# szemenyeim/DynEnv

Hardware: AMD Instinct MI355X
Metric: agent-steps/s (higher is better)
Workload: dtype f64

## Files before the change

### dynenv_amd/csrc/dev_common.h

```cpp
#pragma once
#include <hip/hip_runtime.h>
#include <stdint.h>

#include "dynenv.h"
#include "dynenv_math.h"

#define DE_WAVE 64
#define DE_DEV __device__ __forceinline__
#define DE_OOL static __device__ __noinline__
#define DE_HD __host__ __device__ __forceinline__

struct V2 {
  double x, y;
};
DE_HD V2 v2(double x, double y) { V2 r; r.x = x; r.y = y; return r; }
DE_HD V2 vadd(V2 a, V2 b) { return v2(a.x + b.x, a.y + b.y); }
DE_HD V2 vsub(V2 a, V2 b) { return v2(a.x - b.x, a.y - b.y); }
DE_HD V2 vneg(V2 a) { return v2(-a.x, -a.y); }
DE_HD V2 vmul(V2 a, double s) { return v2(a.x * s, a.y * s); }
DE_HD double vdot(V2 a, V2 b) { return a.x * b.x + a.y * b.y; }
DE_HD double vcross(V2 a, V2 b) { return a.x * b.y - a.y * b.x; }
DE_HD V2 vperp(V2 a) { return v2(-a.y, a.x); }
DE_HD V2 vrotate(V2 a, V2 b) { return v2(a.x * b.x - a.y * b.y, a.x * b.y + a.y * b.x); }
DE_HD double vdot_f(V2 a, V2 b) { return dms_dot(a.x, a.y, b.x, b.y); }
DE_HD V2 vrotate_f(V2 n, V2 j) { return v2(dms_rotate_x(n.x, n.y, j.x, j.y), dms_rotate_y(n.x, n.y, j.x, j.y)); }
DE_HD double vlensq(V2 a) { return vdot(a, a); }
DE_HD V2 vlerp(V2 a, V2 b, double t) { return vadd(vmul(a, 1.0 - t), vmul(b, t)); }
DE_HD double vlen(V2 v) { return dm_sqrt(v.x * v.x + v.y * v.y); }
DE_HD V2 vrot_angle(V2 v, double a) {
  double s, c;
  dm_sincos(a, &s, &c);
  return v2(v.x * c - v.y * s, v.x * s + v.y * c);
}
DE_HD double fmax_cp(double a, double b) { return (a > b) ? a : b; }
DE_HD double fmin_cp(double a, double b) { return (a < b) ? a : b; }
DE_HD double fclamp_cp(double f, double lo, double hi) { return fmin_cp(fmax_cp(f, lo), hi); }
DE_HD double fclamp01_cp(double f) { return fmax_cp(0.0, fmin_cp(f, 1.0)); }

DE_DEV uint64_t wave_ballot(bool p) { return __ballot(p); }
DE_DEV int lane_id() { return (int)__builtin_amdgcn_mbcnt_hi(~0u, __builtin_amdgcn_mbcnt_lo(~0u, 0u)); }
DE_DEV int fresh_lane() {
  int l;
  asm volatile("v_mbcnt_lo_u32_b32 %0, -1, 0\n\tv_mbcnt_hi_u32_b32 %0, -1, %0" : "=v"(l));
  return l;
}
DE_DEV uint64_t lanemask_lt() { return (1ull << lane_id()) - 1ull; }

DE_DEV int bcast_i(int v, int src) { return __builtin_amdgcn_readlane(v, __builtin_amdgcn_readfirstlane(src)); }
DE_DEV double bcast_d(double v, int src) {
  union { double d; int i[2]; } u;
  u.d = v;
  src = __builtin_amdgcn_readfirstlane(src);
  u.i[0] = __builtin_amdgcn_readlane(u.i[0], src);
  u.i[1] = __builtin_amdgcn_readlane(u.i[1], src);
  return u.d;
}
DE_DEV int lane_read_i(int v, int src) { return __builtin_amdgcn_ds_bpermute(src << 2, v); }
DE_DEV double lane_read_d(double v, int src) {
  union { double d; int i[2]; } u;
  u.d = v;
  u.i[0] = __builtin_amdgcn_ds_bpermute(src << 2, u.i[0]);
  u.i[1] = __builtin_amdgcn_ds_bpermute(src << 2, u.i[1]);
  return u.d;
}
DE_DEV int uniform_i(int v) { return __builtin_amdgcn_readfirstlane(v); }
DE_DEV uint64_t uniform_u64(uint64_t v) {
  uint32_t lo = (uint32_t)__builtin_amdgcn_readfirstlane((int)(uint32_t)v);
  uint32_t hi = (uint32_t)__builtin_amdgcn_readfirstlane((int)(uint32_t)(v >> 32));
  return ((uint64_t)hi << 32) | lo;
}
template <typename T>
DE_DEV T* uniform_ptr(T* p) { return (T*)uniform_u64((uint64_t)p); }
DE_DEV double uniform_d(double v) { return __longlong_as_double((long long)uniform_u64((uint64_t)__double_as_longlong(v))); }

struct DevSC {
  double s, c;
};
DE_OOL DevSC dev_sincos(double x) {
  DevSC r;
  dm_sincos(x, &r.s, &r.c);
  return r;
}
DE_OOL DevSC dev_sincos_v(double x) {
  DevSC r;
  dm_sincos_f(x, &r.s, &r.c);
  return r;
}
DE_DEV DevSC dev_sincos_inl(double x) {
  DevSC r;
  dm_sincos(x, &r.s, &r.c);
  return r;
}
DE_OOL double dev_atan2(double y, double x) { return dm_atan2(y, x); }
__device__ const double g_atanTab[30] = DM_ATAN_TAB;
#define DEV_ATAN_TAB_INIT(dst, lane) do { if ((lane) < 30) (dst)[lane] = g_atanTab[lane]; } while (0)
DE_DEV int dev_lds_addr(const void* p) { return (int)(size_t)(const __attribute__((address_space(3))) void*)p; }
DE_OOL double dev_atan2_t(double y, double x, int tab) {
  typedef double __attribute__((ext_vector_type(2))) d2;
  const double aq = __builtin_fabs(y / x);
  typedef const __attribute__((address_space(3))) d2* lds_d2p;
  const lds_d2p row = (lds_d2p)(size_t)(unsigned)(tab + 48 * dm_atan_row(aq));
  const d2 n = row[0], d = row[1], hl = row[2];
  return dm_atan2_finish(y, x, aq, dm_atan_core(aq, n.x, n.y, d.x, d.y, hl.x, hl.y));
}
DE_DEV double dev_cos(double x) { return dev_sincos(x).c; }

#define DE_DBL_MIN 2.2250738585072014e-308
#define DE_COLLISION_SLOP 0.1
#define DE_CONTACT_BIAS_COEF 0.061259621561307376
#define DE_PIVOT_BIAS_COEF 0.022762779044189331
#define DE_JOINT_BIAS_COEF DE_CONTACT_BIAS_COEF
#define DE_DT 0.01
```

### dynenv_amd/csrc/driving_kernels.hip

```cpp
#include "driving_dev.h"

__constant__ DrvConst C;

#include "driving_host.h"

struct DrvMailbox {
  double p1x[DRV_NS][2], p1y[DRV_NS][2], p2x[DRV_NS][2], p2y[DRV_NS][2], nx[DRV_NS], ny[DRV_NS];
  int hash[DRV_NS][2], count[DRV_NS], flag[DRV_NS];
};
struct DrvObsStage {
  float carRow[DRV_MAXA][8];
  float goal[DRV_MAXA][2];
  float shared[DRV_MAXO * 4 + DRV_MAXP * 2 + DRV_LANE_ROWS * 5];
};
#ifdef DRV_PROFILE
#define DRV_PROF(...) __VA_ARGS__
#else
#define DRV_PROF(...)
#endif
#define DRV_CLIST 128
struct __align__(16) DrvLds {
  double px[DRV_NB], py[DRV_NB], vx[DRV_NB], vy[DRV_NB], ang[DRV_NB], w[DRV_NB], vbx[DRV_NB], vby[DRV_NB], wb[DRV_NB];
  double minv[DRV_NB], iinv[DRV_NB];
  double rc[16], rs[16], rotAng[16];
// ... 73 lines not shown
    double relAngle = cosRel * dist;
    pos = relAngle < 0.0 ? LP_InRightLane : LP_InOpposingLane;
  }
  return pos;
}

DE_DEV bool drv_is_off_road(V2 point) {
  int position = LP_OffRoad;
  int rp = road_pos<0>(point, RoadK<0>::cosDir0);
  if (rp < position) position = rp;
  rp = road_pos<1>(point, RoadK<1>::cosDir0);
  if (rp < position) position = rp;
  return position >= LP_OverRoad;
}
DE_DEV bool drv_is_out(V2 p) { return p.x <= 0.0 || p.y <= 0.0 || p.x >= DRV_W || p.y >= DRV_H; }

DE_DEV void apply_friction(double& vx, double& vy, double& w, double m, double friction, double rotFriction,
                           double spin) {
  vx = vx * 1.0 + (0.0 + 0.0) * DE_DT;
  vy = vy * 1.0 + (0.0 + 0.0) * DE_DT;
  w = w * 1.0 + 0.0;
  double factor = friction * m;
  double rotFactor = rotFriction * m;
  double x = vx, y = vy;
  double length = 1.0 / (dm_abs(x) + dm_abs(y) + 1e-5);
  double theta = w;
  double a0 = x * factor * length;
  double a1 = y * factor * length;
  a0 += a1 * spin * theta;
  a1 -= a0 * spin * theta;
  if (dm_abs(x) < factor) x = 0.0; else x -= a0;
  if (dm_abs(y) < factor) y = 0.0; else y -= a1;
  if (dm_abs(theta) < rotFactor) theta = 0.0; else theta -= (theta > 0.0 ? rotFactor : -rotFactor);
  vx = x; vy = y; w = theta;
}

DE_DEV void velocity_update(DrvLds& L, int lane, bool isCar, bool isPed) {
  if (!(isCar || isPed)) return;
  double vx = L.vx[lane], vy = L.vy[lane], w = L.w[lane];
  const int f = L.flags[lane];
  double m, fr, rfr;
  bool dflt = false;
  if (isCar) { m = L.cmass[lane]; fr = CF_FRIC(f) ? 5e-4 : 5e-5; rfr = CF_FRIC(f) ? 2e-5 : 1e-5; }
  else { m = 90.0; fr = 5e-2; rfr = 2e-4; dflt = !PF_DEAD(f); }
  if (dflt) { vx = vx * 1.0 + (0.0 + 0.0) * DE_DT; vy = vy * 1.0 + (0.0 + 0.0) * DE_DT; w = w * 1.0 + 0.0; }
  else apply_friction(vx, vy, w, m, fr, rfr, 0.0);
  L.vx[lane] = vx; L.vy[lane] = vy; L.w[lane] = w;
}
DE_OOL void velocity_update_ool(int nCarPed) {
  const int lane = lane_id(), A = uniform_i(nCarPed) & 0xFF, nPed = uniform_i(nCarPed) >> 8;
  velocity_update(g_L, lane, lane < A, lane >= DRV_SLOT_PED && lane < DRV_SLOT_PED + nPed);
}

struct CarRot { double c, s, cosRel0; };
template <bool INL = false>
DE_DEV CarRot car_refresh_rot(DrvLds& L, int lane, double ang) {
  const DevSC sc = INL ? dev_sincos_inl(ang) : dev_sincos(ang);
  CarRot r;
  r.c = sc.c; r.s = sc.s;
  r.cosRel0 = INL ? dev_sincos_inl(RoadK<0>::dirAngle - ang).c : dev_cos(RoadK<0>::dirAngle - ang);
  L.rc[lane] = r.c; L.rs[lane] = r.s; L.rotAng[lane] = ang; L.cosRel0[lane] = r.cosRel0;
  static_assert(RoadK<1>::dirAngle == 0.0, "cos(road1.dirAngle - angle) is read from rc");
  return r;
}

struct BoxW {
  V2 v[4], n[4];
};
DE_DEV void box_world(BoxW& b, V2 p, double rc, double rs, double hx, double hy) {
  const double lx[4] = {-hx, hx, hx, -hx}, ly[4] = {-hy, -hy, hy, hy};
  const double nx[4] = {-1.0, 0.0, 1.0, 0.0}, ny[4] = {0.0, -1.0, 0.0, 1.0};
#pragma unroll
  for (int i = 0; i < 4; ++i) {
    b.v[i] = v2(dms_xform_x(rc, rs, lx[i], ly[i], p.x), dms_xform_y(rc, rs, lx[i], ly[i], p.y));
    b.n[i] = v2(rc * nx[i] - rs * ny[i], rs * nx[i] + rc * ny[i]);
  }
}

struct Contacts {
  int count;
  V2 n, p1[2], p2[2];
  int hash[2];
};

struct EdgeW {
  V2 ap, bp, n;
  int ah, bh;
};

DE_DEV V2 sel4(const V2* a, int i) {
  V2 r = a[0];
  r = (i == 1) ? a[1] : r;
  r = (i == 2) ? a[2] : r;
  r = (i == 3) ? a[3] : r;
  return r;
}

struct BoxP {
  V2 p;
  double c, s, hx, hy;
};
DE_DEV V2 boxp_vertex(const BoxP& b, int i) {
  const double lx = (i == 1 || i == 2) ? b.hx : -b.hx;
  const double ly = (i >= 2) ? b.hy : -b.hy;
  return v2(dms_xform_x(b.c, b.s, lx, ly, b.p.x), dms_xform_y(b.c, b.s, lx, ly, b.p.y));
}
DE_DEV V2 boxp_normal(const BoxP& b, int i) {
  const double nx = (i == 0) ? -1.0 : ((i == 2) ? 1.0 : 0.0);
  const double ny = (i == 1) ? -1.0 : ((i == 3) ? 1.0 : 0.0);
  return v2(b.c * nx - b.s * ny, b.s * nx + b.c * ny);
}

template <int S> DE_DEV double quad_bcast(double x) {
  int lo = __double2loint(x), hi = __double2hiint(x);
  lo = __builtin_amdgcn_update_dpp(lo, lo, S * 0x55, 0xF, 0xF, false);
  hi = __builtin_amdgcn_update_dpp(hi, hi, S * 0x55, 0xF, 0xF, false);
  return __hiloint2double(hi, lo);
}
DE_DEV void quad_argmax_first(double v, double& best, int& idx) {
  best = -INFINITY; idx = 0;
  double m;
  m = quad_bcast<0>(v); if (m > best) { best = m; idx = 0; }
  m = quad_bcast<1>(v); if (m > best) { best = m; idx = 1; }
  m = quad_bcast<2>(v); if (m > best) { best = m; idx = 2; }
  m = quad_bcast<3>(v); if (m > best) { best = m; idx = 3; }
}

DE_DEV int poly_support_index(const BoxP& p, V2 n, int q) {
  double mx;
  int index;
  quad_argmax_first(vdot_f(boxp_vertex(p, q), n), mx, index);
  return index;
}

DE_DEV EdgeW support_edge_poly(const BoxP& p, int slot, V2 n, int q) {
  int i1 = poly_support_index(p, n, q);
  int i0 = (i1 + 3) & 3;
  int i2 = (i1 + 1) & 3;
  int h = slot * 4;
  V2 n1 = boxp_normal(p, i1), n2 = boxp_normal(p, i2);
  EdgeW e;
  V2 vm = boxp_vertex(p, i1);
  if (vdot(n, n1) > vdot(n, n2)) {
    e.ap = boxp_vertex(p, i0); e.ah = h + i0; e.bp = vm; e.bh = h + i1; e.n = n1;
  } else {
    e.ap = vm; e.ah = h + i1; e.bp = boxp_vertex(p, i2); e.bh = h + i2; e.n = n2;
  }
  return e;
}

DE_DEV int hash_pair(int a, int b) { return 1 + ((a << 8) | b); }

DE_DEV void contact_points(const EdgeW& e1, const EdgeW& e2, V2 n, Contacts& out) {
  double d_e1_a = vcross(e1.ap, n), d_e1_b = vcross(e1.bp, n);
  double d_e2_a = vcross(e2.ap, n), d_e2_b = vcross(e2.bp, n);
  double e1_denom = 1.0 / (d_e1_b - d_e1_a + DE_DBL_MIN);
  double e2_denom = 1.0 / (d_e2_b - d_e2_a + DE_DBL_MIN);
  out.n = n;
  out.count = 0;
  {
    V2 p1 = vadd(vmul(n, 0.0), vlerp(e1.ap, e1.bp, fclamp01_cp((d_e2_b - d_e1_a) * e1_denom)));
    V2 p2 = vadd(vmul(n, -0.0), vlerp(e2.ap, e2.bp, fclamp01_cp((d_e1_a - d_e2_a) * e2_denom)));
    double dist = vdot(vsub(p2, p1), n);
    if (dist <= 0.0) { out.p1[0] = p1; out.p2[0] = p2; out.hash[0] = hash_pair(e1.ah, e2.bh); out.count = 1; }
  }
  {
    V2 p1 = vadd(vmul(n, 0.0), vlerp(e1.ap, e1.bp, fclamp01_cp((d_e2_a - d_e1_a) * e1_denom)));
    V2 p2 = vadd(vmul(n, -0.0), vlerp(e2.ap, e2.bp, fclamp01_cp((d_e1_b - d_e2_a) * e2_denom)));
    double dist = vdot(vsub(p2, p1), n);
    if (dist <= 0.0) {
      int h = hash_pair(e1.bh, e2.ah);
      if (out.count == 0) { out.p1[0] = p1; out.p2[0] = p2; out.hash[0] = h; }
      else { out.p1[1] = p1; out.p2[1] = p2; out.hash[1] = h; }
      out.count += 1;
    }
  }
}

DE_DEV double sat_max_sep(const BoxP& a, const BoxP& b, int q, int& best) {
  const V2 n = boxp_normal(a, q);
  const double d0 = vdot_f(n, boxp_vertex(a, q));
  double minv = INFINITY;
#pragma unroll
  for (int j = 0; j < 4; ++j) {
    double d = vdot_f(n, boxp_vertex(b, j)) - d0;
    if (d < minv) minv = d;
  }
  double maxsep;
  quad_argmax_first(minv, maxsep, best);
  return maxsep;
}

DE_DEV void poly_to_poly(const BoxP& p1, int slot1, const BoxP& p2, int slot2, int q, Contacts& out) {
  out.count = 0;
  int ia, ib;
  double sa = sat_max_sep(p1, p2, q, ia);
  if (sa > 0.0) return;
  double sb = sat_max_sep(p2, p1, q, ib);
  if (sb > 0.0) return;
  V2 n;
  if (sa >= sb) n = boxp_normal(p1, ia); else n = vneg(boxp_normal(p2, ib));
  const EdgeW e1 = support_edge_poly(p1, slot1, n, q);
  const EdgeW e2 = support_edge_poly(p2, slot2, vneg(n), q);
  contact_points(e1, e2, n, out);
}

DE_DEV void circle_to_poly(V2 c, double r, const BoxP& poly, int q, Contacts& out) {
  out.count = 0;
  double maxsep;
  int best;
  const V2 vq = boxp_vertex(poly, q);
  quad_argmax_first(vdot(boxp_normal(poly, q), vsub(c, vq)), maxsep, best);
  if (maxsep > r) return;
  if (maxsep <= 0.0) {
    V2 fn = boxp_normal(poly, best);
    V2 n = vneg(fn);
    V2 pb = vsub(c, vmul(fn, maxsep));
    out.n = n; out.p1[0] = vadd(c, vmul(n, r)); out.p2[0] = pb; out.hash[0] = 0; out.count = 1;
  } else {
    const V2 a = boxp_vertex(poly, (q + 3) & 3), b = vq;
    const V2 d = vsub(b, a);
    const double t = fclamp01_cp(vdot(d, vsub(c, a)) / vlensq(d));
    const V2 pt = vadd(a, vmul(d, t));
    const double dsq = vlensq(vsub(pt, c));
    double bestd = INFINITY;
    V2 bestp = c;
    double m;
    m = quad_bcast<0>(dsq); if (m < bestd) { bestd = m; bestp = v2(quad_bcast<0>(pt.x), quad_bcast<0>(pt.y)); }
    m = quad_bcast<1>(dsq); if (m < bestd) { bestd = m; bestp = v2(quad_bcast<1>(pt.x), quad_bcast<1>(pt.y)); }
    m = quad_bcast<2>(dsq); if (m < bestd) { bestd = m; bestp = v2(quad_bcast<2>(pt.x), quad_bcast<2>(pt.y)); }
    m = quad_bcast<3>(dsq); if (m < bestd) { bestd = m; bestp = v2(quad_bcast<3>(pt.x), quad_bcast<3>(pt.y)); }
    if (bestd <= r * r) {
      double dist = dm_sqrt(bestd);
      V2 delta = vsub(bestp, c);
      V2 n = (dist != 0.0) ? vmul(delta, 1.0 / dist) : vneg(boxp_normal(poly, best));
      out.n = n; out.p1[0] = vadd(c, vmul(n, r)); out.p2[0] = bestp; out.hash[0] = 0; out.count = 1;
    }
  }
}

struct BodyV {
  V2 p, v, vb;
  double w, wb, minv, iinv;
};
DE_DEV V2 static_pos(const DrvLds& L, int idx) {
  if (idx >= DRV_SLOT_BLD) {
    int k = idx - DRV_SLOT_BLD;
    return v2((k & 2) ? 1385.0 : 365.0, (k & 1) ? 800.0 : 200.0);
  }
  return v2(L.ox[idx - DRV_SLOT_OBST], L.oy[idx - DRV_SLOT_OBST]);
}
DE_DEV void body_load(const DrvLds& L, int idx, BodyV& b) {
  const bool dyn = idx < DRV_SLOT_OBST;
  const int bi = dyn ? idx : DRV_SLOT_OBST , oi = (idx >= DRV_SLOT_OBST && idx < DRV_SLOT_BLD) ? idx - DRV_SLOT_OBST : 0;
  const double dpx = L.px[bi], dpy = L.py[bi], sox = L.ox[oi], soy = L.oy[oi];
  const int k = idx - DRV_SLOT_BLD;
// ... 373 lines not shown
    const V2 jl = vmul(n, dj);                                                              \
    const V2 jj = biasLane ? jl : jr;                                                       \
    apply_impulse(a, vneg(jj), r1[q]);                                                      \
    apply_impulse(b, jj, r2[q]);                                                            \
  }
  for (int t = 0; t < nSteps; ++t) {
    if (active && t == due && passes < 10) {
      a.v = v2(fX[ra], fY[ra]); a.w = fW[ra];
      b.v = v2(fX[rb], fY[rb]); b.w = fW[rb];
      DRV_SPLIT_PASS(0)
      if (count > 1) DRV_SPLIT_PASS(1)
      fX[wa] = a.v.x; fY[wa] = a.v.y; fW[wa] = a.w;
      fX[wb_] = b.v.x; fY[wb_] = b.v.y; fW[wb_] = b.w;
      due += period; ++passes;
    }
    __syncthreads();
  }
#undef DRV_SPLIT_PASS
  DrvSplitRet r;
  r.jt0 = jt0; r.jt1 = jt1; r.pk = pk; r.pair = pair; r.bits = bits3;
  r.jn0 = acc[0]; r.jn1 = acc[1];
  r.jb0 = lane_read_d(acc[0], (lane + 32) & 63); r.jb1 = lane_read_d(acc[1], (lane + 32) & 63);
  return r;
}

DRV_PROF(__device__ unsigned long long g_dbgw[4096 * 12];)
DRV_PROF(__device__ unsigned long long g_dbgp[4096 * 8];)
DRV_PROF(__device__ unsigned long long g_dbgr[16];)
DRV_PROF(__device__ unsigned long long g_dbgl[4096 * 8];)
DRV_PROF(__device__ unsigned long long g_dbgs[4096 * 8];)
DRV_PROF(DE_DEV int prof_any(int v) { const uint64_t m = wave_ballot(v != 0); return m ? bcast_i(v, __builtin_ctzll(m)) : 0; })
#ifndef DRV_CONTACT_INLINE
#define DRV_CONTACT_INLINE __forceinline__
#endif

DE_OOL int drv_prestep_solve(int lane, int nCarPed, int pk, int a_pair, int bodyA, int bodyB, int myLevel,
                                             int maxLevel_, int anyActive_, double jn0, double jn1, double jt0, double jt1) {
  DrvLds& L = g_L;
  DrvMailbox& M = L.u.mb;
  int a_state = pk & 0xFF;
  int a_count = (pk >> 8) & 0xFF, a_age = (pk >> 16) & 0xFF;
  bool touched = (pk >> 24) & 1, freeMe = (pk >> 25) & 1, hashSame = (pk >> 26) & 1, prevInert = (pk >> 27) & 1;
  bool skipped = (pk >> 28) & 1, slotOcc = (pk >> 29) & 1, active = (pk >> 30) & 1;
  const bool isCar = lane < (uniform_i(nCarPed) & 0xFF), isPed = lane >= DRV_SLOT_PED && lane < DRV_SLOT_PED + (uniform_i(nCarPed) >> 8);
  const int maxLevel = (int)(signed char)(uniform_i(maxLevel_) & 0xFF), period = uniform_i(maxLevel_) >> 8;
  const uint64_t activeMask = uniform_i(anyActive_) ? 1ull : 0ull;
DRV_PROF(const unsigned long long P0 = __builtin_amdgcn_s_memtime();)
  double jn[2] = {jn0, jn1}, jt[2] = {jt0, jt1};
  V2 n = v2(0.0, 0.0), r1[2], r2[2];
  r1[0] = r1[1] = r2[0] = r2[1] = v2(0.0, 0.0);
  double nMass[2] = {0.0, 0.0}, tMass[2] = {0.0, 0.0}, bias[2] = {0.0, 0.0}, bounce[2] = {0.0, 0.0}, jBias[2] = {0.0, 0.0};
  const double arb_e = 0.05 * 0.05, arb_u = 0.0 * 0.0;
  bool restIn = false;
  if (active) {
    BodyV a, b;
    body_load(L, bodyA, a);
    body_load(L, bodyB, b);
    restIn = a.v.x == 0.0 && a.v.y == 0.0 && a.w == 0.0 && b.v.x == 0.0 && b.v.y == 0.0 && b.w == 0.0;
    r1[0] = vsub(v2(M.p1x[lane][0], M.p1y[lane][0]), a.p);
    r2[0] = vsub(v2(M.p2x[lane][0], M.p2y[lane][0]), b.p);
    if (a_count > 1) {
      r1[1] = vsub(v2(M.p1x[lane][1], M.p1y[lane][1]), a.p);
      r2[1] = vsub(v2(M.p2x[lane][1], M.p2y[lane][1]), b.p);
    }
    n = v2(M.nx[lane], M.ny[lane]);
    V2 body_delta = vsub(b.p, a.p);
#pragma unroll
    for (int c = 0; c < 2; ++c) {
      if (c == 0 || a_count > 1) {
        nMass[c] = 1.0 / (k_scalar_body(a, r1[c], n) + k_scalar_body(b, r2[c], n));
        double dist = vdot_f(vadd(vsub(r2[c], r1[c]), body_delta), n);
        bias[c] = -DE_CONTACT_BIAS_COEF * fmin_cp(0.0, dist + DE_COLLISION_SLOP) / DE_DT;
        jBias[c] = 0.0;
        bounce[c] = vdot_f(relative_velocity(a, b, r1[c], r2[c]), n) * arb_e;
      }
    }
  }
  __syncthreads();
DRV_PROF(const unsigned long long P1 = __builtin_amdgcn_s_memtime();)

  velocity_update(L, lane, isCar, isPed);
DRV_PROF(int profMode = 0; const unsigned long long P2 = __builtin_amdgcn_s_memtime();)
  bool tookSplit = false;
  if (activeMask && maxLevel == 0) {
    __syncthreads();
    if (active) {
      BodyV a, b;
      body_load(L, bodyA, a);
      body_load(L, bodyB, b);
      if (a_state != ARB_FIRST) arb_warm_start(a, b, n, r1, r2, jn, jt, a_count);
      if (wave_ballot(!arb_is_bias_only(a, b, jn, jt, bounce, a_count)) == 0ull) {
DRV_PROF(profMode = 1;)
#pragma unroll 1
        for (int iter = 0; iter < 10; ++iter)
          if (wave_ballot(arb_apply_bias_only(a, b, n, r1, r2, nMass, bias, jBias, a_count)) == 0ull) break;
      } else {
DRV_PROF(profMode = 2;)
#pragma unroll 1
        for (int iter = 0; iter < 10; ++iter) arb_apply_impulse(a, b, n, r1, r2, nMass, tMass, bias, bounce, jBias, jn, jt, a_count, arb_u);
      }
      body_store_vel(L, bodyA, a);
      body_store_vel(L, bodyB, b);
    }
    __syncthreads();
  } else if (activeMask) {
    __syncthreads();
    for (int lv = 0; lv <= maxLevel; ++lv) {
      if (active && myLevel == lv && a_state != ARB_FIRST) {
        BodyV a, b;
        body_load(L, bodyA, a);
        body_load(L, bodyB, b);
        arb_warm_start(a, b, n, r1, r2, jn, jt, a_count);
        body_store_vel(L, bodyA, a);
        body_store_vel(L, bodyB, b);
      }
      __syncthreads();
    }
    BodyV a, b;
    bool biasOnly = true;
    if (active) {
      body_load(L, bodyA, a); body_load(L, bodyB, b);
      biasOnly = arb_is_bias_only(a, b, jn, jt, bounce, a_count);
    }
    const int nSteps = maxLevel + 1 + period * 9;
    int due = myLevel, passes = 0;
DRV_PROF(profMode = wave_ballot(!biasOnly) == 0ull ? 3 : 4;)
    if (wave_ballot(!biasOnly) == 0ull) {
      const int ra = body_rd(bodyA), rb = body_rd(bodyB), wa = body_wr(bodyA), wb_ = body_wr(bodyB);
      for (int t = 0; t < nSteps; ++t) {
// ... 325 lines not shown
      uint64_t who = wave_ballot(active && rank == k);
      if (who == 0ull) continue;
      int b = __builtin_ctzll(who);
      const int ab = bcast_i(bodyAB, b), ba = ab & 0xFF, bb2 = ab >> 8;
      const int pa = ba < DRV_SLOT_OBST ? bcast_i(bl, ba) : 0, pb = bb2 < DRV_SLOT_OBST ? bcast_i(bl, bb2) : 0;
      const int la = pa & 0xFF, lb = pb & 0xFF;
      int lv = la > lb ? la : lb;
      const int fa = (pa >> 8) - 1, fb = (pb >> 8) - 1;
      const int lo = fa < 0 ? fb : (fb < 0 ? fa : (fa < fb ? fa : fb));
      if (lo >= 0 && lv - lo + 1 > period) period = lv - lo + 1;
      if (lane == b) myLevel = lv;
      if (lane == ba || lane == bb2) bl = (lv + 1) | (((bl >> 8) ? (bl >> 8) : lv + 1) << 8);
      maxLevel = lv > maxLevel ? lv : maxLevel;
    }
    if (lane < DRV_NS) L.sLevel[lane] = (unsigned char)myLevel;
    if (lane == 0) L.sLvMeta = (maxLevel & 0xFF) | (period << 8);
  }

DRV_PROF(const unsigned long long T2 = __builtin_amdgcn_s_memtime();)
DRV_PROF(if (lane == 0 && blockIdx.x < 4096) { unsigned long long* d = g_dbgs + blockIdx.x * 8; d[0] += U1 - T1; d[1] += U2 - U1; d[2] += U3 - U2; d[3] += U4 - U3; d[4] += T2 - U4; })
  const int solveBits = drv_prestep_solve(lane, nCarPed,
                                          (a_state & 0xFF) | ((a_count & 0xFF) << 8) | ((a_age & 0xFF) << 16) | (touched ? 1 << 24 : 0) | (freeMe ? 1 << 25 : 0) |
                                              (hashSame ? 1 << 26 : 0) | (prevInert ? 1 << 27 : 0) | (skipped ? 1 << 28 : 0) | (slotOcc ? 1 << 29 : 0) | (active ? 1 << 30 : 0),
                                          a_pair, bodyA, bodyB, myLevel, (maxLevel & 0xFF) | (period << 8), activeMask != 0ull ? 1 : 0, jn[0], jn[1], jt[0], jt[1]);
  occ &= ~freeMask;
DRV_PROF(const unsigned long long T3 = T2, T4 = T2, T5 = __builtin_amdgcn_s_memtime(); const int profModeW = (uniform_i(solveBits) >> 4) & 7;)
DRV_PROF(if (lane == 0 && blockIdx.x < 4096) { unsigned long long* d = g_dbgp + blockIdx.x * 8; d[0] += T1 - T0; d[1] += T2 - T1; d[2] += T3 - T2; d[3] += T4 - T3; d[4] += T5 - T4; d[5] += 1ull + (light ? (1ull << 16) : 0ull); d[6] += (unsigned long long)(maxLevel + 1) + ((unsigned long long)(maxLevel + 1) << (12 * profModeW)); d[7] += (unsigned long long)nTouched + ((unsigned long long)profCand << 16); })
  {
    ContactRet ret;
    ret.occ = occ; ret.err = err | (uniform_i(solveBits) & 6) | ((uniform_i(solveBits) & 8) << 1);
    return ret;
  }
}

DE_OOL int drv_partial_obs_fused(PvIn in, uint64_t seed, int A, int* envi, int env_id_offset, int e, int nPedObst, int elapsed,
                                 uint32_t episode, int noiseTypeAgents, double magn, float* __restrict__ obs, int budgetCycles);
#ifndef DRV_DEFER_MIN_CONTACT
#define DRV_DEFER_MIN_CONTACT 5
#endif
#ifndef DRV_PV_DEADLINE_PCT
#define DRV_PV_DEADLINE_PCT 110
#endif
#ifndef DRV_FUSED_AGENTS
#define DRV_FUSED_AGENTS 10
#endif
struct DrvLightRet {
  int cand, dirty, bits;
};
struct DrvSeedOnly { uint64_t seed; };
DE_OOL DrvLightRet drv_light_substep(int it_, int lane, int A_, int nPed_, int nObst_, int elapsed_,
                                                      uint32_t seedLo, uint32_t seedHi, uint32_t genv_, uint32_t episode_, int stateBits) {
  DrvLds& L = g_L;
DRV_PROF(const unsigned long long Q0 = __builtin_amdgcn_s_memtime();)
  const int lastCand = L.lastCand[lane];
  const int it = uniform_i(it_), A = uniform_i(A_), nPed = uniform_i(nPed_), nObst = uniform_i(nObst_), elapsed = uniform_i(elapsed_);
  const uint32_t genv = (uint32_t)uniform_i((int)genv_), episode = (uint32_t)uniform_i((int)episode_);
  DrvSeedOnly S;
  S.seed = ((uint64_t)(uint32_t)uniform_i((int)seedHi) << 32) | (uint64_t)(uint32_t)uniform_i((int)seedLo);
  const bool isCar = lane < A;
  const bool isPed = lane >= DRV_SLOT_PED && lane < DRV_SLOT_PED + nPed;
  const bool isBody = isCar || isPed;
  const bool vbValid = (uniform_i(stateBits) & 1) != 0;
  bool aabbValid = (uniform_i(stateBits) & 2) != 0;
    bool turned = false;
    const int bi = lane & (DRV_NB - 1), ci = lane & 15;
    int f = L.flags[bi];
    double px = L.px[bi], py = L.py[bi], vx = L.vx[bi], vy = L.vy[bi], ang = L.ang[bi];
    const double w = L.w[bi];
    const double vbx = vbValid ? L.vbx[bi] : 0.0, vby = vbValid ? L.vby[bi] : 0.0, wb = vbValid ? L.wb[bi] : 0.0;
    double rcv = L.rc[ci], rsv = L.rs[ci], rotAngv = L.rotAng[ci], cosRel0v = L.cosRel0[ci];
    const double goalx = L.goalx[ci], goaly = L.goaly[ci], dprev = L.dprev[ci], chx = L.chx[ci], chy = L.chy[ci];
    double rew = L.rewAcc[ci], posrew = L.posAcc[ci];
    int moving = L.moving[bi];
    if (!isBody) { f = 0; px = 0.0; py = 0.0; vx = 0.0; vy = 0.0; }
    if (isCar) {
      if (it == 0) {
        const int actPk = (int)L.act[lane];
        const int acc = (actPk & 3) - 1, steer = ((actPk >> 2) - 1) * 2;
        if (!CF_FIN(f)) {
          double dirx = L.dirx[lane], diry = L.diry[lane];
          double power = (double)acc;
          double moveDir = vx * dirx + vy * diry;
          bool skip = false;
          if (acc < 0) power = (double)acc * 0.75;
          if (acc == 0) power = (moveDir == 0.0) ? 0.0 : (moveDir > 0.0 ? -2.0 : 2.0);
          else if (acc < 0 && moveDir > 0.0) skip = true;
          else if (acc > 0 && moveDir < 0.0) skip = true;
          if (!skip) {
            const double cs = rcv, sn = rsv;
            const double cpower = L.cpower[lane];
            vx = vx + cpower * power * cs;
            vy = vy + cpower * power * sn;
            if (acc == 0 && (vx * dirx + vy * diry) * moveDir < 0.0) { vx = 0.0; vy = 0.0; }
          }
          if (steer != 0) {
            const double rot = (double)steer * (DM_PI / 180.0);
            ang = ang + rot;
            const DevSC rsc = dev_sincos_inl(rot);
            const double sn = rsc.s, cs = rsc.c;
            const double dx = dirx * cs - diry * sn, dy = dirx * sn + diry * cs;
            L.dirx[lane] = dx; L.diry[lane] = dy;
            const double nvx = vx * cs - vy * sn, nvy = vx * sn + vy * cs;
            vx = nvx; vy = nvy;
            L.ang[lane] = ang;
            const CarRot cr = car_refresh_rot<true>(L, lane, ang);
            rcv = cr.c; rsv = cr.s; rotAngv = ang; cosRel0v = cr.cosRel0;
            turned = true;
          }
        }
      }
    }
DRV_PROF(const unsigned long long Q1 = __builtin_amdgcn_s_memtime();)
    const V2 pos = v2(px, py);
    int lp = LP_OffRoad;
    if (isBody) {
      int rp = road_pos<0>(pos, isCar ? cosRel0v : RoadK<0>::cosDir0);
      if (rp < lp) lp = rp;
      rp = road_pos<1>(pos, isCar ? rcv : RoadK<1>::cosDir0);
      if (rp < lp) lp = rp;
    }
DRV_PROF(const unsigned long long Q2 = __builtin_amdgcn_s_memtime();)
    if (isCar) {
      const double dnow = vlen(vsub(pos, v2(goalx, goaly)));
      const double diff = dprev - dnow;
      if (!CF_FIN(f)) { const double d50 = diff / 50.0; rew += d50; posrew += dm_max(0.0, d50); }
      L.prevx[lane] = px; L.prevy[lane] = py; L.dprev[lane] = dnow;
      if (lp >= LP_OverRoad) {
        if (!CF_FIN(f)) {
          if (lp == LP_OverRoad && dnow < 100.0) {
            lp = LP_AtGoal;
            f |= (1 << 4) | (1 << 6);
            rew += (double)(DRV_MAX_TIME - elapsed) / 100.0;
            posrew += (double)(DRV_MAX_TIME - elapsed) / 100.0;
          } else {
            f |= CF_CRASH_BITS;
            rew -= vlen(v2(vx, vy)) / 5.0;
          }
        }
      } else if (lp == LP_InOpposingLane) {
        if (!CF_FIN(f)) rew -= vlen(v2(vx, vy)) / 10000.0;
      }
      f = CF_SET_LP(f, lp);
      if (px >= DRV_W + 50.0 || px <= -50.0 || py >= DRV_H + 50.0 || py <= -50.0) { vx = 0.0; vy = 0.0; }
      L.flags[lane] = f;
      L.vx[lane] = vx; L.vy[lane] = vy;
      L.rewAcc[lane] = rew; L.posAcc[lane] = posrew;
DRV_PROF(asm volatile("" ::: "memory");)
    } else if (isPed) {
      if (!PF_DEAD(f)) {
        int crossing = PF_CROSSING(f), beginc = PF_BEGIN(f), side = PF_SIDE(f);
        const bool isOffRoad = lp >= LP_OverRoad;
        const bool isOut = drv_is_out(pos);
        if (moving > 0) {
          moving = (moving - DRV_TIME_DIFF > 0) ? moving - DRV_TIME_DIFF : 0;
          if (crossing) {
            if (!beginc && isOffRoad) { moving = 0; crossing = 0; vx = 0.0; vy = 0.0; }
            else if (beginc && !isOffRoad) { beginc = 0; }
          }
          if (isOut) { moving = 0; vx = 0.0; vy = 0.0; }
        } else {
          if (!crossing) {
            dm_u32x4 u = dm_env_rng(S.seed, genv, episode, DM_RNG_PED_MOVE, (uint32_t)(lane - DRV_SLOT_PED), (uint32_t)elapsed);
            const bool r1 = PF_ROAD(f) != 0;
            const V2 rdir = r1 ? v2(RoadK<1>::dirx, RoadK<1>::diry) : v2(RoadK<0>::dirx, RoadK<0>::diry);
            const V2 rnrm = r1 ? v2(RoadK<1>::nx, RoadK<1>::ny) : v2(RoadK<0>::nx, RoadK<0>::ny);
            V2 dir = rdir;
            moving = dm_randint(u.v[0], 5000, 30000);
            int speed = dm_randint(u.v[1], -2, 2);
            if (!isOffRoad) {
              crossing = 1; beginc = 0;
              if (speed == 0) speed = 2;
            } else if (isOut) {
              dir = drv_is_out(vadd(pos, rdir)) ? vneg(rdir) : rdir;
            } else if (dm_unit(u.v[2]) < 0.05) {
              crossing = 1; beginc = 1;
              dir = side ? rnrm : vneg(rnrm);
              side = side ? 0 : 1;
              speed = dm_randint(u.v[3], 1, 2);
            }
            const V2 nv = vmul(vmul(dir, (double)PF_SPEED(f)), (double)speed);
            vx = nv.x; vy = nv.y;
          } else if (isOffRoad) {
            crossing = 0; beginc = 0;
          }
        }
        L.moving[lane] = moving;
        L.flags[lane] = PEDF_PACK(PF_ROAD(f), side, 0, crossing, beginc, PF_SPEED(f));
        L.vx[lane] = vx; L.vy[lane] = vy;
      }
    }

DRV_PROF(const unsigned long long Q3 = __builtin_amdgcn_s_memtime();)
    double bl = 0.0, bb = 0.0, br = -1.0, bt = -1.0;
    bool live = false;
    int sj = 3;
    if (isBody) {
      const double npx = px + (vx + vbx) * DE_DT, npy = py + (vy + vby) * DE_DT, nang = ang + (w + wb) * DE_DT;
      const bool still = !turned && vx == 0.0 && vy == 0.0 && w == 0.0 && vbx == 0.0 && vby == 0.0 && wb == 0.0;
      L.px[lane] = npx; L.py[lane] = npy; L.ang[lane] = nang;
      const bool frozen = !turned && vx == 0.0 && vy == 0.0 && w == 0.0 && npx == px && npy == py && nang == ang;
      sj = (still ? 1 : 0) | (frozen ? 2 : 0);
      L.still[lane] = sj;
      live = true;
      if (isCar) {
        if (nang != rotAngv) { const CarRot cr = car_refresh_rot<true>(L, lane, nang); rcv = cr.c; rsv = cr.s; }
        if (!aabbValid || !frozen) {
          BoxW bw;
          box_world(bw, v2(npx, npy), rcv, rsv, chx, chy);
          double l = INFINITY, r = -INFINITY, b = INFINITY, t = -INFINITY;
#pragma unroll
          for (int k = 0; k < 4; ++k) {
            l = fmin_cp(l, bw.v[k].x); r = fmax_cp(r, bw.v[k].x); b = fmin_cp(b, bw.v[k].y); t = fmax_cp(t, bw.v[k].y);
          }
          bl = l - 0.0; bb = b - 0.0; br = r + 0.0; bt = t + 0.0;
          L.aabb[lane][0] = bl; L.aabb[lane][1] = bb; L.aabb[lane][2] = br; L.aabb[lane][3] = bt;
        } else {
          bl = L.aabb[lane][0]; bb = L.aabb[lane][1]; br = L.aabb[lane][2]; bt = L.aabb[lane][3];
        }
      } else {
        bl = npx - 5.0; bb = npy - 5.0; br = npx + 5.0; bt = npy + 5.0;
      }
    } else if (lane >= DRV_SLOT_OBST && lane < DRV_SLOT_BLD + 4) {
      live = lane >= DRV_SLOT_BLD || (lane - DRV_SLOT_OBST) < nObst;
      const V2 c = static_pos(L, lane);
      const double ex = lane >= DRV_SLOT_BLD ? 400.0 : 10.0, ey = lane >= DRV_SLOT_BLD ? 225.0 : 10.0;
      bl = -ex + c.x; br = ex + c.x; bb = -ey + c.y; bt = ey + c.y;
    }
    aabbValid = true;
    __syncthreads();
DRV_PROF(const unsigned long long Q4 = __builtin_amdgcn_s_memtime();)

    int cand = 0;
    bool candMoving = false, removed = false;
    int dirty = 0;
    {
      const int carStill = (int)(wave_ballot(isCar && (sj & 1)) & 0x3FFull);
      const int carFrozen = (int)(wave_ballot(isCar && (sj & 2)) & 0x3FFull);
#pragma unroll
      for (int i = 0; i < DRV_MAXA; ++i) {
        const double al = L.aabb[i][0], ab = L.aabb[i][1], ar = L.aabb[i][2], at = L.aabb[i][3];
        const bool hit = (al <= br) & (bl <= ar) & (ab <= bt) & (bb <= at);
        cand |= hit ? (1 << i) : 0;
      }
      {
        const int lim = lane < A ? lane : A;
        cand &= live ? ((1 << lim) - 1) : 0;
      }
      if (cand) candMoving = !(sj & 1) || (cand & ~carStill) != 0;
      const int clean = (lastCand >= 0 && (sj & 2)) ? (cand & lastCand & carFrozen) : 0;
      dirty = cand & ~clean;
      removed = lastCand < 0 || (lastCand & ~cand) != 0;
    }
  L.lastCand[lane] = cand;
DRV_PROF(if (lane == 0 && blockIdx.x < 4096) { unsigned long long* d = g_dbgl + blockIdx.x * 8; const unsigned long long Q5 = __builtin_amdgcn_s_memtime(); if (it == 0) { for (int k = 0; k < 8; ++k) d[k] = 0ull; } d[0] += Q1 - Q0; d[1] += Q2 - Q1; d[2] += Q3 - Q2; d[3] += Q4 - Q3; d[4] += Q5 - Q4; d[5] += Q5 - Q0; })
  DrvLightRet ret;
  ret.cand = cand; ret.dirty = dirty; ret.bits = (candMoving ? 1 : 0) | (removed ? 2 : 0) | (cand != lastCand ? 4 : 0);
  return ret;
}
DE_DEV unsigned drv_hw_simd_key() {
  const unsigned hw = (unsigned)__builtin_amdgcn_s_getreg(63492) , xcc = (unsigned)__builtin_amdgcn_s_getreg(63508) ;
  return ((xcc & 0xFu) << 16) | (hw & 0xFF30u);
}
DE_DEV int drv_launch_tick(const DrvState& S) { return S.tick_src ? uniform_i(__atomic_load_n(&S.iso[13], __ATOMIC_RELAXED)) : S.tick; }
DE_DEV int drv_launch_pv(const DrvState& S) { return S.tick_src ? uniform_i(__atomic_load_n(&S.iso[14], __ATOMIC_RELAXED)) : S.pv_par; }
DE_DEV int drv_iso_assign(const DrvState& S, int lane, int tick) {
  const int b = blockIdx.x, E = S.E;
  if (!S.iso_on) return b;
  const int buf = tick % 3;
  if (b == 0 && lane == 0) { const int nn = (tick + 2) % 3; S.iso[nn] = 0; S.iso[3 + nn] = 0; }
  if (S.iso_on == 3) return b;
  int K = uniform_i(S.iso[buf]);
  const int cap = S.iso_on == 1 ? DRV_ISO_MAX : DRV_ISO_LIST;
  K = K < cap ? K : cap;
  const int G = S.iso_on == 1 ? 4 * DRV_ISO_GROUPS : E;
  if (S.iso_on == 1) {
    if (b < G) { if (lane == 0) S.iso_hw[(size_t)(tick & 1) * (4 * DRV_ISO_GROUPS) + b] = drv_hw_simd_key(); }
    else if (b == G + 3 * DRV_ISO_MAX) {
      const unsigned* hw = S.iso_hw + (size_t)((tick + 1) & 1) * (4 * DRV_ISO_GROUPS);
      bool bad = false;
      for (int g = DRV_ISO_G0 + lane; g < DRV_ISO_G0 + DRV_ISO_GSPAN; g += 64) {
        const unsigned k0 = hw[g], k1 = hw[g + DRV_ISO_GROUPS], k2 = hw[g + 2 * DRV_ISO_GROUPS], k3 = hw[g + 3 * DRV_ISO_GROUPS];
        bad |= k0 == 0xFFFFFFFFu || k0 != k1 || k0 != k2 || k0 != k3;
      }
      const bool ok = wave_ballot(bad) == 0ull;
// ... 520 lines not shown
```

Baseline: 260.8 million.

## Spread car trig and contact pre-solve across idle wave halves via permlane swaps

Adds permlane32/16 swap helpers and uses them to hand the second sincos argument (road-relative angle, steer rotation) to otherwise idle lanes, so one inline sincos per lane replaces two serial ones. The per-contact pre-solve work for the second contact point moves to mirror lanes 32+, halving the serial work per slot. SAT and support-edge code now take each box's quad vertex once and broadcast it instead of recomputing vertices, and the lastCand load is moved later. This adds lane-shuffle traffic, wave-wide ballots and cross-lane dependencies, and it assumes at most 32 slots and car lanes inside the first row/half.

Result: no change. 260.5 million (-0.1%).

```diff
diff --git a/dynenv_amd/csrc/dev_common.h b/dynenv_amd/csrc/dev_common.h
--- a/dynenv_amd/csrc/dev_common.h
+++ b/dynenv_amd/csrc/dev_common.h
@@ -63,6 +63,27 @@
   u.i[1] = __builtin_amdgcn_ds_bpermute(src << 2, u.i[1]);
   return u.d;
 }
+DE_DEV double half_put_d(double keep, double send) {
+  const int lo = (int)__builtin_amdgcn_permlane32_swap((unsigned)__double2loint(keep), (unsigned)__double2loint(send), false, false)[0];
+  const int hi = (int)__builtin_amdgcn_permlane32_swap((unsigned)__double2hiint(keep), (unsigned)__double2hiint(send), false, false)[0];
+  return __hiloint2double(hi, lo);
+}
+DE_DEV double half_get_d(double v) {
+  const int lo = (int)__builtin_amdgcn_permlane32_swap((unsigned)__double2loint(v), (unsigned)__double2loint(v), false, false)[1];
+  const int hi = (int)__builtin_amdgcn_permlane32_swap((unsigned)__double2hiint(v), (unsigned)__double2hiint(v), false, false)[1];
+  return __hiloint2double(hi, lo);
+}
+DE_DEV double row_put_d(double keep, double send) {
+  const int lo = (int)__builtin_amdgcn_permlane16_swap((unsigned)__double2loint(keep), (unsigned)__double2loint(send), false, false)[0];
+  const int hi = (int)__builtin_amdgcn_permlane16_swap((unsigned)__double2hiint(keep), (unsigned)__double2hiint(send), false, false)[0];
+  return __hiloint2double(hi, lo);
+}
+DE_DEV double row_get_d(double v) {
+  const int lo = (int)__builtin_amdgcn_permlane16_swap((unsigned)__double2loint(v), (unsigned)__double2loint(v), false, false)[1];
+  const int hi = (int)__builtin_amdgcn_permlane16_swap((unsigned)__double2hiint(v), (unsigned)__double2hiint(v), false, false)[1];
+  return __hiloint2double(hi, lo);
+}
+DE_DEV int half_put_i(int keep, int send) { return (int)__builtin_amdgcn_permlane32_swap((unsigned)keep, (unsigned)send, false, false)[0]; }
 DE_DEV int uniform_i(int v) { return __builtin_amdgcn_readfirstlane(v); }
 DE_DEV uint64_t uniform_u64(uint64_t v) {
   uint32_t lo = (uint32_t)__builtin_amdgcn_readfirstlane((int)(uint32_t)v);
diff --git a/dynenv_amd/csrc/driving_kernels.hip b/dynenv_amd/csrc/driving_kernels.hip
--- a/dynenv_amd/csrc/driving_kernels.hip
+++ b/dynenv_amd/csrc/driving_kernels.hip
@@ -149,16 +149,10 @@
   velocity_update(g_L, lane, lane < A, lane >= DRV_SLOT_PED && lane < DRV_SLOT_PED + nPed);
 }
 
-struct CarRot { double c, s, cosRel0; };
-template <bool INL = false>
-DE_DEV CarRot car_refresh_rot(DrvLds& L, int lane, double ang) {
-  const DevSC sc = INL ? dev_sincos_inl(ang) : dev_sincos(ang);
-  CarRot r;
-  r.c = sc.c; r.s = sc.s;
-  r.cosRel0 = INL ? dev_sincos_inl(RoadK<0>::dirAngle - ang).c : dev_cos(RoadK<0>::dirAngle - ang);
-  L.rc[lane] = r.c; L.rs[lane] = r.s; L.rotAng[lane] = ang; L.cosRel0[lane] = r.cosRel0;
+DE_DEV void car_refresh_rot(DrvLds& L, int lane, double ang) {
+  const DevSC sc = dev_sincos(ang);
+  L.rc[lane] = sc.c; L.rs[lane] = sc.s; L.rotAng[lane] = ang; L.cosRel0[lane] = dev_cos(RoadK<0>::dirAngle - ang);
   static_assert(RoadK<1>::dirAngle == 0.0, "cos(road1.dirAngle - angle) is read from rc");
-  return r;
 }
 
 struct BoxW {
@@ -223,15 +217,15 @@
   m = quad_bcast<3>(v); if (m > best) { best = m; idx = 3; }
 }
 
-DE_DEV int poly_support_index(const BoxP& p, V2 n, int q) {
+DE_DEV int poly_support_index(V2 vq, V2 n) {
   double mx;
   int index;
-  quad_argmax_first(vdot_f(boxp_vertex(p, q), n), mx, index);
+  quad_argmax_first(vdot_f(vq, n), mx, index);
   return index;
 }
 
-DE_DEV EdgeW support_edge_poly(const BoxP& p, int slot, V2 n, int q) {
-  int i1 = poly_support_index(p, n, q);
+DE_DEV EdgeW support_edge_poly(const BoxP& p, V2 vq, int slot, V2 n) {
+  int i1 = poly_support_index(vq, n);
   int i0 = (i1 + 3) & 3;
   int i2 = (i1 + 1) & 3;
   int h = slot * 4;
@@ -274,15 +268,17 @@
   }
 }
 
-DE_DEV double sat_max_sep(const BoxP& a, const BoxP& b, int q, int& best) {
+DE_DEV double sat_max_sep(const BoxP& a, V2 aq, V2 bq, int q, int& best) {
   const V2 n = boxp_normal(a, q);
-  const double d0 = vdot_f(n, boxp_vertex(a, q));
+  const double d0 = vdot_f(n, aq);
   double minv = INFINITY;
-#pragma unroll
-  for (int j = 0; j < 4; ++j) {
-    double d = vdot_f(n, boxp_vertex(b, j)) - d0;
-    if (d < minv) minv = d;
-  }
+#define DRV_SAT_VERTEX(j)                                                                 \
+  {                                                                                       \
+    double d = vdot_f(n, v2(quad_bcast<j>(bq.x), quad_bcast<j>(bq.y))) - d0;              \
+    if (d < minv) minv = d;                                                               \
+  }
+  DRV_SAT_VERTEX(0) DRV_SAT_VERTEX(1) DRV_SAT_VERTEX(2) DRV_SAT_VERTEX(3)
+#undef DRV_SAT_VERTEX
   double maxsep;
   quad_argmax_first(minv, maxsep, best);
   return maxsep;
@@ -290,15 +286,16 @@
 
 DE_DEV void poly_to_poly(const BoxP& p1, int slot1, const BoxP& p2, int slot2, int q, Contacts& out) {
   out.count = 0;
+  const V2 v1q = boxp_vertex(p1, q), v2q = boxp_vertex(p2, q);
   int ia, ib;
-  double sa = sat_max_sep(p1, p2, q, ia);
+  double sa = sat_max_sep(p1, v1q, v2q, q, ia);
   if (sa > 0.0) return;
-  double sb = sat_max_sep(p2, p1, q, ib);
+  double sb = sat_max_sep(p2, v2q, v1q, q, ib);
   if (sb > 0.0) return;
   V2 n;
   if (sa >= sb) n = boxp_normal(p1, ia); else n = vneg(boxp_normal(p2, ib));
-  const EdgeW e1 = support_edge_poly(p1, slot1, n, q);
-  const EdgeW e2 = support_edge_poly(p2, slot2, vneg(n), q);
+  const EdgeW e1 = support_edge_poly(p1, v1q, slot1, n);
+  const EdgeW e2 = support_edge_poly(p2, v2q, slot2, vneg(n));
   contact_points(e1, e2, n, out);
 }
 
@@ -778,29 +775,37 @@
   double nMass[2] = {0.0, 0.0}, tMass[2] = {0.0, 0.0}, bias[2] = {0.0, 0.0}, bounce[2] = {0.0, 0.0}, jBias[2] = {0.0, 0.0};
   const double arb_e = 0.05 * 0.05, arb_u = 0.0 * 0.0;
   bool restIn = false;
-  if (active) {
-    BodyV a, b;
-    body_load(L, bodyA, a);
-    body_load(L, bodyB, b);
-    restIn = a.v.x == 0.0 && a.v.y == 0.0 && a.w == 0.0 && b.v.x == 0.0 && b.v.y == 0.0 && b.w == 0.0;
-    r1[0] = vsub(v2(M.p1x[lane][0], M.p1y[lane][0]), a.p);
-    r2[0] = vsub(v2(M.p2x[lane][0], M.p2y[lane][0]), b.p);
-    if (a_count > 1) {
-      r1[1] = vsub(v2(M.p1x[lane][1], M.p1y[lane][1]), a.p);
-      r2[1] = vsub(v2(M.p2x[lane][1], M.p2y[lane][1]), b.p);
-    }
-    n = v2(M.nx[lane], M.ny[lane]);
-    V2 body_delta = vsub(b.p, a.p);
-#pragma unroll
-    for (int c = 0; c < 2; ++c) {
-      if (c == 0 || a_count > 1) {
-        nMass[c] = 1.0 / (k_scalar_body(a, r1[c], n) + k_scalar_body(b, r2[c], n));
-        double dist = vdot_f(vadd(vsub(r2[c], r1[c]), body_delta), n);
-        bias[c] = -DE_CONTACT_BIAS_COEF * fmin_cp(0.0, dist + DE_COLLISION_SLOP) / DE_DT;
-        jBias[c] = 0.0;
-        bounce[c] = vdot_f(relative_velocity(a, b, r1[c], r2[c]), n) * arb_e;
-      }
-    }
+  {
+    static_assert(DRV_NS <= 32, "slot s mirrors to lane s + 32");
+    const bool mirror = lane >= 32;
+    const int sl = lane & 31, cI = mirror ? 1 : 0;
+    const int mine = active && a_count > 1 ? (bodyA | (bodyB << 8) | (1 << 16)) : 0;
+    const int work = half_put_i(active ? (bodyA | (bodyB << 8) | (1 << 16)) : 0, mine);
+    double nMassC = 0.0, biasC = 0.0, bounceC = 0.0;
+    if (work != 0) {
+      BodyV a, b;
+      body_load(L, work & 0xFF, a);
+      body_load(L, (work >> 8) & 0xFF, b);
+      restIn = a.v.x == 0.0 && a.v.y == 0.0 && a.w == 0.0 && b.v.x == 0.0 && b.v.y == 0.0 && b.w == 0.0;
+      const V2 r1c = vsub(v2(M.p1x[sl][cI], M.p1y[sl][cI]), a.p);
+      const V2 r2c = vsub(v2(M.p2x[sl][cI], M.p2y[sl][cI]), b.p);
+      n = v2(M.nx[sl], M.ny[sl]);
+      if (!mirror) {
+        r1[0] = r1c; r2[0] = r2c;
+        if (a_count > 1) {
+          r1[1] = vsub(v2(M.p1x[sl][1], M.p1y[sl][1]), a.p);
+          r2[1] = vsub(v2(M.p2x[sl][1], M.p2y[sl][1]), b.p);
+        }
+      }
+      V2 body_delta = vsub(b.p, a.p);
+      nMassC = 1.0 / (k_scalar_body(a, r1c, n) + k_scalar_body(b, r2c, n));
+      double dist = vdot_f(vadd(vsub(r2c, r1c), body_delta), n);
+      biasC = -DE_CONTACT_BIAS_COEF * fmin_cp(0.0, dist + DE_COLLISION_SLOP) / DE_DT;
+      bounceC = vdot_f(relative_velocity(a, b, r1c, r2c), n) * arb_e;
+    }
+    nMass[0] = nMassC; bias[0] = biasC; bounce[0] = bounceC;
+    nMass[1] = half_get_d(nMassC); bias[1] = half_get_d(biasC); bounce[1] = half_get_d(bounceC);
+    restIn = restIn && !mirror;
   }
   __syncthreads();
 DRV_PROF(const unsigned long long P1 = __builtin_amdgcn_s_memtime();)
@@ -1232,7 +1237,6 @@
                                                       uint32_t seedLo, uint32_t seedHi, uint32_t genv_, uint32_t episode_, int stateBits) {
   DrvLds& L = g_L;
 DRV_PROF(const unsigned long long Q0 = __builtin_amdgcn_s_memtime();)
-  const int lastCand = L.lastCand[lane];
   const int it = uniform_i(it_), A = uniform_i(A_), nPed = uniform_i(nPed_), nObst = uniform_i(nObst_), elapsed = uniform_i(elapsed_);
   const uint32_t genv = (uint32_t)uniform_i((int)genv_), episode = (uint32_t)uniform_i((int)episode_);
   DrvSeedOnly S;
@@ -1253,40 +1257,43 @@
     double rew = L.rewAcc[ci], posrew = L.posAcc[ci];
     int moving = L.moving[bi];
     if (!isBody) { f = 0; px = 0.0; py = 0.0; vx = 0.0; vy = 0.0; }
-    if (isCar) {
-      if (it == 0) {
-        const int actPk = (int)L.act[lane];
-        const int acc = (actPk & 3) - 1, steer = ((actPk >> 2) - 1) * 2;
-        if (!CF_FIN(f)) {
-          double dirx = L.dirx[lane], diry = L.diry[lane];
-          double power = (double)acc;
-          double moveDir = vx * dirx + vy * diry;
-          bool skip = false;
-          if (acc < 0) power = (double)acc * 0.75;
-          if (acc == 0) power = (moveDir == 0.0) ? 0.0 : (moveDir > 0.0 ? -2.0 : 2.0);
-          else if (acc < 0 && moveDir > 0.0) skip = true;
-          else if (acc > 0 && moveDir < 0.0) skip = true;
-          if (!skip) {
-            const double cs = rcv, sn = rsv;
-            const double cpower = L.cpower[lane];
-            vx = vx + cpower * power * cs;
-            vy = vy + cpower * power * sn;
-            if (acc == 0 && (vx * dirx + vy * diry) * moveDir < 0.0) { vx = 0.0; vy = 0.0; }
-          }
-          if (steer != 0) {
-            const double rot = (double)steer * (DM_PI / 180.0);
-            ang = ang + rot;
-            const DevSC rsc = dev_sincos_inl(rot);
-            const double sn = rsc.s, cs = rsc.c;
-            const double dx = dirx * cs - diry * sn, dy = dirx * sn + diry * cs;
-            L.dirx[lane] = dx; L.diry[lane] = dy;
-            const double nvx = vx * cs - vy * sn, nvy = vx * sn + vy * cs;
-            vx = nvx; vy = nvy;
-            L.ang[lane] = ang;
-            const CarRot cr = car_refresh_rot<true>(L, lane, ang);
-            rcv = cr.c; rsv = cr.s; rotAngv = ang; cosRel0v = cr.cosRel0;
-            turned = true;
-          }
+    if (it == 0) {
+      const int actPk = isCar ? (int)L.act[ci] : (1 | (1 << 2));
+      const int acc = (actPk & 3) - 1, steer = ((actPk >> 2) - 1) * 2;
+      double dirx = 0.0, diry = 0.0;
+      if (isCar && !CF_FIN(f)) {
+        dirx = L.dirx[lane]; diry = L.diry[lane];
+        double power = (double)acc;
+        double moveDir = vx * dirx + vy * diry;
+        bool skip = false;
+        if (acc < 0) power = (double)acc * 0.75;
+        if (acc == 0) power = (moveDir == 0.0) ? 0.0 : (moveDir > 0.0 ? -2.0 : 2.0);
+        else if (acc < 0 && moveDir > 0.0) skip = true;
+        else if (acc > 0 && moveDir < 0.0) skip = true;
+        if (!skip) {
+          const double cs = rcv, sn = rsv;
+          const double cpower = L.cpower[lane];
+          vx = vx + cpower * power * cs;
+          vy = vy + cpower * power * sn;
+          if (acc == 0 && (vx * dirx + vy * diry) * moveDir < 0.0) { vx = 0.0; vy = 0.0; }
+        }
+      }
+      const bool steers = isCar && !CF_FIN(f) && steer != 0;
+      if (wave_ballot(steers) != 0ull) {
+        const double rot = steers ? (double)steer * (DM_PI / 180.0) : 0.0;
+        const double angT = ang + rot;
+        const DevSC sc = dev_sincos_inl(half_put_d(row_put_d(angT, rot), RoadK<0>::dirAngle - angT));
+        const double cs = row_get_d(sc.c), sn = row_get_d(sc.s), cr0 = half_get_d(sc.c);
+        if (steers) {
+          ang = angT;
+          const double dx = dirx * cs - diry * sn, dy = dirx * sn + diry * cs;
+          L.dirx[lane] = dx; L.diry[lane] = dy;
+          const double nvx = vx * cs - vy * sn, nvy = vx * sn + vy * cs;
+          vx = nvx; vy = nvy;
+          L.ang[lane] = ang;
+          L.rc[lane] = sc.c; L.rs[lane] = sc.s; L.rotAng[lane] = ang; L.cosRel0[lane] = cr0;
+          rcv = sc.c; rsv = sc.s; rotAngv = ang; cosRel0v = cr0;
+          turned = true;
         }
       }
     }
@@ -1374,16 +1381,24 @@
     double bl = 0.0, bb = 0.0, br = -1.0, bt = -1.0;
     bool live = false;
     int sj = 3;
+    const double npx = px + (vx + vbx) * DE_DT, npy = py + (vy + vby) * DE_DT, nang = ang + (w + wb) * DE_DT;
+    const bool frozen = !turned && vx == 0.0 && vy == 0.0 && w == 0.0 && npx == px && npy == py && nang == ang;
+    const bool rotMoved = isCar && nang != rotAngv;
+    if (wave_ballot(rotMoved) != 0ull) {
+      const DevSC sc = dev_sincos_inl(half_put_d(nang, RoadK<0>::dirAngle - nang));
+      const double cr0 = half_get_d(sc.c);
+      if (rotMoved) {
+        rcv = sc.c; rsv = sc.s;
+        L.rc[lane] = sc.c; L.rs[lane] = sc.s; L.rotAng[lane] = nang; L.cosRel0[lane] = cr0;
+      }
+    }
     if (isBody) {
-      const double npx = px + (vx + vbx) * DE_DT, npy = py + (vy + vby) * DE_DT, nang = ang + (w + wb) * DE_DT;
       const bool still = !turned && vx == 0.0 && vy == 0.0 && w == 0.0 && vbx == 0.0 && vby == 0.0 && wb == 0.0;
       L.px[lane] = npx; L.py[lane] = npy; L.ang[lane] = nang;
-      const bool frozen = !turned && vx == 0.0 && vy == 0.0 && w == 0.0 && npx == px && npy == py && nang == ang;
       sj = (still ? 1 : 0) | (frozen ? 2 : 0);
       L.still[lane] = sj;
       live = true;
       if (isCar) {
-        if (nang != rotAngv) { const CarRot cr = car_refresh_rot<true>(L, lane, nang); rcv = cr.c; rsv = cr.s; }
         if (!aabbValid || !frozen) {
           BoxW bw;
           box_world(bw, v2(npx, npy), rcv, rsv, chx, chy);
@@ -1410,6 +1425,7 @@
     __syncthreads();
 DRV_PROF(const unsigned long long Q4 = __builtin_amdgcn_s_memtime();)
 
+    const int lastCand = L.lastCand[lane];
     int cand = 0;
     bool candMoving = false, removed = false;
     int dirty = 0;
```
